# VitorMPCastro/MessyerRaytracer

Measured on AMD Instinct MI355X. Metric: Mrays/s (primary, closest-hit), higher is better.
Workload: dtype f32

## Files before the change

### messyerraytracer_amd/csrc/packet_rows_kernel.h

```cpp
#pragma once

#define RA_LMINX "s20"
#define RA_LMINY "s21"
#define RA_LMINZ "s22"
#define RA_LREF "s23"
#define RA_LMAXX "s24"
#define RA_LMAXY "s25"
#define RA_LMAXZ "s26"
#define RA_RREF "s27"
#define RA_RMINX "s28"
#define RA_RMINY "s29"
#define RA_RMINZ "s30"
#define RA_RMAXX "s32"
#define RA_RMAXY "s33"
#define RA_RMAXZ "s34"
#define RA_MASK "s[60:61]"
#define RA_MASKLO "s60"
#define RA_MASKHI "s61"
#define RA_V0X "s20"
#define RA_V0Y "s21"
#define RA_V0Z "s22"
#define RA_ID "s23"
#define RA_E1X "s24"
#define RA_E1Y "s25"
// ... 179 lines not shown
	"s_branch L_" P "done_%=\n"                                                                                     \
	"L_" P "tri_%=:\n"                                                                                              \
	MRT_ROWS_TRI_STEP(P, RS, POPBIT, CNT_T, ANYHIT_CODE)                                                             \
	"L_" P "done_%=:\n"

#define MRT_ROWS_POP_ISSUE(P, POPBITNO, V0123)                                                                      \
	"s_bitcmp1_b32 %[ev], " POPBITNO "\n"                                                                           \
	"s_cbranch_scc0 L_" P "pi_%=\n"                                                                                 \
	"v_add_u32 " MRT_OP("sp", P) ", -16, " MRT_OP("sp", P) "\n"                                                     \
	"ds_read_b128 " V0123 ", " MRT_OP("sp", P) "\n"                                                                 \
	"L_" P "pi_%=:\n"
#define MRT_ROWS_POP_TAKE(P, RS, POPBITNO, V0, V2, V3)                                                               \
	"s_bitcmp1_b32 %[ev], " POPBITNO "\n"                                                                           \
	"s_cbranch_scc0 L_" P "pt_%=\n"                                                                                 \
	"v_readfirstlane_b32 " MRT_OP("cur", P) ", " V0 "\n"                                                            \
	"v_readfirstlane_b32 " RS##_MASKLO ", " V2 "\n"                                                                  \
	"v_readfirstlane_b32 " RS##_MASKHI ", " V3 "\n"                                                                  \
	"L_" P "pt_%=:\n"

#define MRT_ROWS_CLOBBERS                                                                                             \
	"vcc", "scc", "s20", "s21", "s22", "s23", "s24", "s25", "s26", "s27", "s28", "s29", "s30", "s31", "s32", "s33", \
	"s34", "s35", "s36", "s37", "s38", "s39", "s40", "s41", "s42", "s43", "s44", "s45", "s46", "s47", "s48", "s49", \
	"s50", "s51", "s52", "s53", "s54", "s55", "s56", "s57", "s58", "s59", "s60", "s61", "s62", "s63", "s64", "s65", \
	"s66", "s67", "v50", "v51", "v52", "v53", "v54", "v55", "v56", "v57", "v58", "v59", "v60"

#define MRT_ROWS_OUT(P, S)                                                                                            \
	[cur##P] "+s"(S.cur), [sp##P] "+v"(S.sp), [lim##P] "+v"(S.lim), [bt##P] "+v"(S.bt), [bu##P] "+v"(S.bu),         \
	[bv##P] "+v"(S.bv), [bs##P] "+v"(S.bs), [bi##P] "+v"(S.bi), [mask##P] "+s"(S.mask)
#define MRT_ROWS_IN(P, S)                                                                                             \
	[ox##P] "v"(S.ox), [oy##P] "v"(S.oy), [oz##P] "v"(S.oz), [dx##P] "v"(S.dx), [dy##P] "v"(S.dy), [dz##P] "v"(S.dz), \
	[tmin##P] "v"(S.tmin), [ix##P] "v"(S.ix), [iy##P] "v"(S.iy), [iz##P] "v"(S.iz), [nrx##P] "v"(S.nrx),            \
	[nry##P] "v"(S.nry), [nrz##P] "v"(S.nrz)

struct PacketRegs {
	float ox, oy, oz, dx, dy, dz, tmin;
	float ix, iy, iz, nrx, nry, nrz;
	float lim;
	float bt, bu, bv;
	uint32_t bs, bi;
	uint32_t sp;
	uint32_t cur;
	unsigned long long mask;
};

#define MRT_ROWS_LOOP1(CNT_N, CNT_T, CNT_P, T_PRE, T_POST, ANYHIT_CODE, BX, BY, BZ)                                          \
	asm volatile(                                                                                                   \
		"s_mov_b64 s[60:61], %[maskA]\n"                                                                            \
		"L_loop_%=:\n"                                                                                              \
		"s_lshl_b32 s52, %[curA], 6\n"                                                                              \
		T_PRE                                                                                                       \
		"s_load_dwordx16 s[20:35], %[rows], s52\n"                                                                  \
		"s_waitcnt lgkmcnt(0)\n"                                                                                    \
		T_POST                                                                                                      \
		MRT_ROWS_STEP("A", RA, "1", CNT_N, CNT_T, CNT_P, ANYHIT_CODE, BX, BY, BZ)                                   \
		"s_cmp_eq_u32 %[ev], 0\n"                                                                                   \
		"s_cbranch_scc1 L_loop_%=\n"                                                                                \
		MRT_ROWS_POP_ISSUE("A", "0", "v[50:53]")                                                                    \
		"s_waitcnt lgkmcnt(0)\n"                                                                                    \
		MRT_ROWS_POP_TAKE("A", RA, "0", "v50", "v52", "v53")                                                        \
		"s_mov_b32 %[ev], 0\n"                                                                                      \
		"s_cmp_lg_u32 %[curA], 0x7fffffff\n"                                                                        \
		"s_cbranch_scc1 L_loop_%=\n"                                                                                \
		"s_waitcnt vmcnt(0)\n"                    \
		"s_mov_b64 %[maskA], s[60:61]\n"                                                                            \
		: MRT_ROWS_OUT(A, a), [ev] "+s"(ev), [cntn] "+s"(cnt_n), [cntt] "+s"(cnt_t), [cntw] "+s"(cnt_w), [cntp] "+s"(sp_max) \
		: MRT_ROWS_IN(A, a), [rows] "s"(rows), [qmask] "s"(qmask), [eps] "s"(eps), [vneg] "v"(vneg)                 \
		: MRT_ROWS_CLOBBERS)

#define MRT_ROWSW_GROUP_SLAB(P, OWN, LM, RM, BX, BY, BZ)                                                              \
	"s_cmp_eq_u64 " OWN ", 0\n"                                                                                     \
	"s_cbranch_scc1 L_" P "skip_%=\n"                             \
	MRT_ROWS_SLAB(P, RA, BX, BY, BZ)                                                                                \
	"v_cmp_le_f32_e64 " LM ", v50, v53\n"                                                                           \
	"v_cmp_le_f32_e64 " RM ", v56, v52\n"                                                                           \
	"L_" P "sdone_%=:\n"
#define MRT_ROWSW_GROUP_SKIP(P, LM, RM)                                                                               \
	"L_" P "skip_%=:\n"                                                                                             \
	"s_mov_b64 " LM ", 0\n"                                                                                         \
	"s_mov_b64 " RM ", 0\n"                                                                                         \
	"s_branch L_" P "sdone_%=\n"

#define MRT_ROWSW_ANYHIT(P) \
	"v_cndmask_b32_e64 " MRT_OP("lim", P) ", " MRT_OP("lim", P) ", %[vneg], s[54:55]\n"
#define MRT_ROWSW_ANYDONE                                                                                             \
	"v_cmp_neq_f32_e64 s[56:57], %[limA], %[vneg]\n"                                                                \
	"v_cmp_neq_f32_e64 s[58:59], %[limB], %[vneg]\n"                                                                \
	"s_or_b64 s[56:57], s[56:57], s[58:59]\n"                                                                       \
	"s_cbranch_scc1 L_goon_%=\n"                                                                                    \
	"s_mov_b32 %[curA], 0x7fffffff\n"                                                                               \
	"s_branch L_exit_%=\n"                                                                                          \
	"L_goon_%=:\n"

#ifndef MRT_ROWS_KPREFETCH
#define MRT_ROWS_KPREFETCH 1
#endif
#if MRT_ROWS_KPREFETCH
#define MRT_ROWSW_KPREFETCH                                                                                           \
	"s_lshl_b32 s48, " RA_LREF ", 6\n"                                                                               \
	"s_lshl_b32 s49, " RA_RREF ", 6\n"                                                                               \
	"s_load_dword s64, %[rows], s48\n"                                                                              \
	"s_load_dword s65, %[rows], s49\n"
#define MRT_ROWSW_FARPREFETCH ""
#else
#define MRT_ROWSW_KPREFETCH ""
#define MRT_ROWSW_FARPREFETCH                                                                                         \
	"v_lshlrev_b32 v55, 6, v54\n"                                       \
	"global_load_dword v60, v55, %[rows]\n"
#endif

#define MRT_ROWS_LOOPW(CNT_N, CNT_T, CNT_P, ANYA, ANYB, ANYDONE, BX, BY, BZ)                                                 \
	asm volatile(                                                                                                   \
		"s_mov_b64 s[60:61], %[maskA]\n"                                                                            \
		"s_mov_b64 s[62:63], %[maskB]\n"                                                                            \
		"L_loop_%=:\n"                                                                                              \
		"s_lshl_b32 s52, %[curA], 6\n"                                                                              \
		"s_load_dwordx16 s[20:35], %[rows], s52\n"                                                                  \
		"s_waitcnt lgkmcnt(0)\n"                                                                                    \
		"s_bitcmp1_b32 %[curA], 31\n"                                                                               \
		"s_cbranch_scc1 L_tri_%=\n"                                                                                 \
		CNT_N                                                                                                       \
		MRT_ROWSW_KPREFETCH                                                                                         \
		MRT_ROWSW_GROUP_SLAB("A", "s[60:61]", "s[36:37]", "s[38:39]", BX, BY, BZ)                                   \
		MRT_ROWSW_GROUP_SLAB("B", "s[62:63]", "s[40:41]", "s[42:43]", BX, BY, BZ)                                   \
		"s_or_b64 s[44:45], s[36:37], s[40:41]\n"                     \
		"s_cbranch_scc0 L_lmiss_%=\n"                                                                               \
		"s_or_b64 vcc, s[38:39], s[42:43]\n"                                              \
		"s_cbranch_scc0 L_onlyl_%=\n"                                                                               \
		      \
		"v_cmp_lt_f32_e64 s[46:47], v50, v56\n"                                           \
		"s_bitcmp1_b32 s46, 0\n"                                                                                    \
		"s_cselect_b32 s53, " RA_RREF ", " RA_LREF "\n"                                                   \
		"s_cselect_b32 %[curA], " RA_LREF ", " RA_RREF "\n"                                               \
		"s_cselect_b64 s[50:51], s[38:39], s[36:37]\n"                 \
		"s_cselect_b64 s[58:59], s[42:43], s[40:41]\n"                                                              \
		"s_cselect_b64 s[60:61], s[36:37], s[38:39]\n"                                        \
		"s_cselect_b64 s[62:63], s[40:41], s[42:43]\n"                                                              \
		"v_mov_b32 v50, s50\n"                                                                                      \
		"v_mov_b32 v51, s51\n"                                                                                      \
		"v_mov_b32 v52, s58\n"                                                                                      \
		"v_mov_b32 v53, s59\n"                                                                                      \
		"v_mov_b32 v54, s53\n"                                                                                      \
		"ds_write_b128 %[spA], v[50:53]\n"                                                                          \
		"ds_write_b32 %[spA], v54 offset:16\n"                                                                      \
		"v_add_u32 %[spA], 32, %[spA]\n"                                                                            \
		CNT_P                                                                                                       \
		MRT_ROWSW_FARPREFETCH                                                                                       \
		"s_branch L_loop_%=\n"                                                                                      \
		"L_onlyl_%=:\n"                                                                                             \
		"s_mov_b32 %[curA], " RA_LREF "\n"                                                                          \
		"s_mov_b64 s[60:61], s[36:37]\n"                                                                            \
		"s_mov_b64 s[62:63], s[40:41]\n"                                                                            \
		"s_branch L_loop_%=\n"                                                                                      \
		"L_lmiss_%=:\n"                                                                                             \
		"s_or_b64 vcc, s[38:39], s[42:43]\n"                                                                        \
		"s_cbranch_scc0 L_pop_%=\n"                                                                                 \
		"s_mov_b32 %[curA], " RA_RREF "\n"                                                                          \
		"s_mov_b64 s[60:61], s[38:39]\n"                                                                            \
		"s_mov_b64 s[62:63], s[42:43]\n"                                                                            \
		"s_branch L_loop_%=\n"                                                                                      \
		"L_tri_%=:\n"                                                                                               \
		CNT_T                                                                                                       \
		"s_cmp_eq_u64 s[60:61], 0\n"                                                                                \
		"s_cbranch_scc1 L_Atnext_%=\n"                                                                              \
		MRT_ROWS_TRI_TEST("A", RA, "s[60:61]", "%[curA]", ANYA)                                                     \
		"s_cmp_eq_u64 s[62:63], 0\n"                                                                                \
		"s_cbranch_scc1 L_Btnext_%=\n"                                                                              \
		MRT_ROWS_TRI_TEST("B", RA, "s[62:63]", "%[curA]", ANYB)                                                     \
		ANYDONE                                                                                                     \
		"s_bitcmp1_b32 " RA_FLAGS ", 0\n"                                       \
		"s_cbranch_scc1 L_pop_%=\n"                                                                                 \
		"s_add_u32 %[curA], %[curA], 1\n"                                                                           \
		"s_branch L_loop_%=\n"                                                                                      \
		"L_pop_%=:\n"                                                                                               \
		"v_add_u32 %[spA], -32, %[spA]\n"                                                                           \
		"ds_read_b128 v[50:53], %[spA]\n"                                                                           \
		"ds_read_b32 v54, %[spA] offset:16\n"                                                                       \
		"s_waitcnt lgkmcnt(0)\n"                                                                                    \
		"v_readfirstlane_b32 %[curA], v54\n"                                                                        \
		"v_readfirstlane_b32 s60, v50\n"                                                                            \
		"v_readfirstlane_b32 s61, v51\n"                                                                            \
		"v_readfirstlane_b32 s62, v52\n"                                                                            \
		"v_readfirstlane_b32 s63, v53\n"                                                                            \
		"s_cmp_lg_u32 %[curA], 0x7fffffff\n"                                                                        \
		"s_cbranch_scc1 L_loop_%=\n"                                                                                \
		"s_branch L_exit_%=\n"                                                                                      \
		MRT_ROWSW_GROUP_SKIP("A", "s[36:37]", "s[38:39]")                                                           \
		MRT_ROWSW_GROUP_SKIP("B", "s[40:41]", "s[42:43]")                                                           \
		"L_exit_%=:\n"                                                                                              \
		"s_waitcnt vmcnt(0)\n"                    \
		"s_mov_b64 %[maskA], s[60:61]\n"                                                                            \
		"s_mov_b64 %[maskB], s[62:63]\n"                                                                            \
		: MRT_ROWS_OUT(A, a), [limB] "+v"(b.lim), [btB] "+v"(b.bt), [buB] "+v"(b.bu), [bvB] "+v"(b.bv),             \
		  [bsB] "+v"(b.bs), [biB] "+v"(b.bi), [maskB] "+s"(b.mask), [cntn] "+s"(cnt_n), [cntt] "+s"(cnt_t), [cntp] "+s"(sp_max) \
		: MRT_ROWS_IN(A, a), MRT_ROWS_IN(B, b), [rows] "s"(rows), [qmask] "s"(qmask), [eps] "s"(eps), [vneg] "v"(vneg) \
		: MRT_ROWS_CLOBBERS)


#define MRT_ROWS_SLAB1(P, RS, SIDE, TE, BX, BY, BZ, MASK)                                                             \
	"v_fma_f32 v51, " MRT_NEAR_##BX(RS, X, SIDE) ", " MRT_OP("ix", P) ", " MRT_OP("nrx", P) "\n"                      \
	"v_fma_f32 v52, " MRT_NEAR_##BY(RS, Y, SIDE) ", " MRT_OP("iy", P) ", " MRT_OP("nry", P) "\n"                      \
	"v_fma_f32 v53, " MRT_NEAR_##BZ(RS, Z, SIDE) ", " MRT_OP("iz", P) ", " MRT_OP("nrz", P) "\n"                      \
	"v_fma_f32 v54, " MRT_FAR_##BX(RS, X, SIDE) ", " MRT_OP("ix", P) ", " MRT_OP("nrx", P) "\n"                       \
	"v_fma_f32 v55, " MRT_FAR_##BY(RS, Y, SIDE) ", " MRT_OP("iy", P) ", " MRT_OP("nry", P) "\n"                       \
	"v_fma_f32 v57, " MRT_FAR_##BZ(RS, Z, SIDE) ", " MRT_OP("iz", P) ", " MRT_OP("nrz", P) "\n"                       \
	"v_max_f32 v53, v53, " MRT_OP("tmin", P) "\n"                                                                   \
	"v_min_f32 v57, v57, " MRT_OP("lim", P) "\n"                                                                    \
	"v_max3_f32 " TE ", v51, v52, v53\n"                                                                            \
	"v_min3_f32 v54, v54, v55, v57\n"                                                                               \
	"v_cmp_le_f32_e64 " MASK ", " TE ", v54\n"

#define MRT_ROWSC_CHILD(SIDE, TE, CULLBITS, MA, MB, BX, BY, BZ)                                                       \
	"s_and_b32 s48, s44, " CULLBITS "\n"                                 \
	"s_cbranch_scc1 L_cull" #SIDE "_%=\n"                                                                           \
	"s_cmp_eq_u64 s[60:61], 0\n"                                                                                    \
	"s_cbranch_scc1 L_" #SIDE "A0_%=\n"                                                                             \
	MRT_ROWS_SLAB1("A", RA, SIDE, TE, BX, BY, BZ, MA)                                                               \
	"L_" #SIDE "A1_%=:\n"                                                                                           \
	"s_cmp_eq_u64 s[62:63], 0\n"                                                                                    \
	"s_cbranch_scc1 L_" #SIDE "B0_%=\n"                                                                             \
	MRT_ROWS_SLAB1("B", RA, SIDE, TE, BX, BY, BZ, MB)                                                               \
	"L_" #SIDE "B1_%=:\n"
#define MRT_ROWSC_CHILD_OOL(SIDE, MA, MB)                                                                             \
	"L_cull" #SIDE "_%=:\n"                                                                                         \
	MRT_ROWSC_CNT_CULL                                                                                              \
	"s_mov_b64 " MA ", 0\n"                                                                                         \
	"s_mov_b64 " MB ", 0\n"                                                                                         \
	"s_branch L_" #SIDE "B1_%=\n"                                                                                   \
	"L_" #SIDE "A0_%=:\n"                                                                                           \
	"s_mov_b64 " MA ", 0\n"                                                                                         \
	"s_branch L_" #SIDE "A1_%=\n"                                                                                   \
	"L_" #SIDE "B0_%=:\n"                                                                                           \
	"s_mov_b64 " MB ", 0\n"                                                                                         \
	"s_branch L_" #SIDE "B1_%=\n"
#define MRT_ROWSC_CNT_CULL ""

#define MRT_ROWSC_VLOAD(VDST, REF)                                                                                   \
	"v_lshl_add_u32 v62, " REF ", 6, %[cvo]\n"                                                                      \
	"global_load_dword " VDST ", v62, %[rows]\n"

#ifndef MRT_ROWSC_KPF
#define MRT_ROWSC_KPF 0
#endif
#if MRT_ROWSC_KPF
#define MRT_ROWSC_KPREFETCH                                                                                           \
	"s_lshl_b32 s46, " RA_LREF ", 6\n"                                                                               \
	"s_lshl_b32 s47, " RA_RREF ", 6\n"                                                                               \
	"s_load_dword s64, %[rows], s46\n"                                                                              \
	"s_load_dword s65, %[rows], s47\n"
#else
#define MRT_ROWSC_KPREFETCH ""
#endif
#define MRT_ROWS_LOOPC(CNT_N, CNT_T, CNT_P, ANYA, ANYB, ANYDONE, BX, BY, BZ)                                          \
	asm volatile(                                                                                                   \
		"s_mov_b64 s[60:61], %[maskA]\n"                                                                            \
		"s_mov_b64 s[62:63], %[maskB]\n"                                                                            \
		"L_vload_%=:\n"                                     \
		MRT_ROWSC_VLOAD("v60", "%[curA]")                                                                           \
		"s_mov_b64 s[66:67], 0\n"                                                                                   \
		"L_loop_%=:\n"                                                                                              \
		"s_lshl_b32 s52, %[curA], 6\n"                                                                              \
		"s_load_dwordx16 s[20:35], %[rows], s52\n"                                                                  \
		"s_waitcnt lgkmcnt(0)\n"                                                                                    \
		"s_bitcmp1_b32 %[curA], 31\n"                                                                               \
		"s_cbranch_scc1 L_tri_%=\n"                                                                                 \
		CNT_N                                                                                                       \
		"s_waitcnt vmcnt(0)\n"                      \
		"v_cndmask_b32_e64 v58, v60, v61, s[66:67]\n"                                                               \
		"v_mul_f32 v58, v58, %[cw]\n"                                                                               \
		MRT_ROWSC_VLOAD("v60", RA_LREF)            \
		"v_add_f32_dpp v59, v58, v58 row_shr:1 row_mask:0xf bank_mask:0xf bound_ctrl:1\n"  \
		MRT_ROWSC_VLOAD("v61", RA_RREF)                                                                             \
		"v_add_f32_dpp v58, v59, v59 row_shr:2 row_mask:0xf bank_mask:0xf bound_ctrl:1\n"                           \
		"s_nop 1\n"                                                                                                 \
		"v_add_f32_dpp v59, v58, v58 row_shr:4 row_mask:0xf bank_mask:0xf bound_ctrl:1\n"                           \
		"v_cmp_lt_f32_e64 s[44:45], v59, %[ccc]\n"  \
		MRT_ROWSC_KPREFETCH                                                                                         \
		"s_or_b32 s44, s44, s45\n"                                                                                  \
		MRT_ROWSC_CHILD(L, "v50", "0x00800080", "s[36:37]", "s[40:41]", BX, BY, BZ)                                 \
// ... 36 lines not shown
		"s_mov_b64 s[62:63], s[42:43]\n"                                                                            \
		"s_mov_b64 s[66:67], -1\n"                                                                                  \
		"s_branch L_loop_%=\n"                                                                                      \
		"L_tri_%=:\n"                                                                                               \
		CNT_T                                                                                                       \
		"s_cmp_eq_u64 s[60:61], 0\n"                                                                                \
		"s_cbranch_scc1 L_Atnext_%=\n"                                                                              \
		MRT_ROWS_TRI_TEST("A", RA, "s[60:61]", "%[curA]", ANYA)                                                     \
		"s_cmp_eq_u64 s[62:63], 0\n"                                                                                \
		"s_cbranch_scc1 L_Btnext_%=\n"                                                                              \
		MRT_ROWS_TRI_TEST("B", RA, "s[62:63]", "%[curA]", ANYB)                                                     \
		ANYDONE                                                                                                     \
		"s_bitcmp1_b32 " RA_FLAGS ", 0\n"                                       \
		"s_cbranch_scc1 L_pop_%=\n"                                                                                 \
		"s_add_u32 %[curA], %[curA], 1\n"                                                                           \
		"s_branch L_loop_%=\n"                                                                                      \
		"L_pop_%=:\n"                                                                                               \
		"v_add_u32 %[spA], -32, %[spA]\n"                                                                           \
		"ds_read_b128 v[50:53], %[spA]\n"                                                                           \
		"ds_read_b32 v54, %[spA] offset:16\n"                                                                       \
		"s_waitcnt lgkmcnt(0)\n"                                                                                    \
		"v_readfirstlane_b32 %[curA], v54\n"                                                                        \
		"v_readfirstlane_b32 s60, v50\n"                                                                            \
		"v_readfirstlane_b32 s61, v51\n"                                                                            \
		"v_readfirstlane_b32 s62, v52\n"                                                                            \
		"v_readfirstlane_b32 s63, v53\n"                                                                            \
		"s_cmp_lg_u32 %[curA], 0x7fffffff\n"                                                                        \
		"s_cbranch_scc1 L_vload_%=\n"                                                                               \
		"s_branch L_exit_%=\n"                                                                                      \
		MRT_ROWSC_CHILD_OOL(L, "s[36:37]", "s[40:41]")                                                              \
		MRT_ROWSC_CHILD_OOL(R, "s[38:39]", "s[42:43]")                                                              \
		"L_exit_%=:\n"                                                                                              \
		"s_waitcnt vmcnt(0)\n"                 \
		"s_mov_b64 %[maskA], s[60:61]\n"                                                                            \
		"s_mov_b64 %[maskB], s[62:63]\n"                                                                            \
		: MRT_ROWS_OUT(A, a), [limB] "+v"(b.lim), [btB] "+v"(b.bt), [buB] "+v"(b.bu), [bvB] "+v"(b.bv),             \
		  [bsB] "+v"(b.bs), [biB] "+v"(b.bi), [maskB] "+s"(b.mask), [cntn] "+s"(cnt_n), [cntt] "+s"(cnt_t), [cntp] "+s"(sp_max) \
		: MRT_ROWS_IN(A, a), MRT_ROWS_IN(B, b), [rows] "s"(rows), [qmask] "s"(qmask),                                \
		  [eps] "s"(eps), [vneg] "v"(vneg), [cw] "v"(cull.w), [ccc] "v"(cull.cc), [cvo] "v"(cull.voff)               \
		: MRT_ROWS_CLOBBERS, "v61", "v62")

struct CullRegs {
	float w;
	float cc;
	uint32_t voff;
};

#define MRT_ROWS_T_PRE "s_memtime s[64:65]\n s_waitcnt lgkmcnt(0)\n"
#define MRT_ROWS_T_POST "s_memtime s[66:67]\n s_waitcnt lgkmcnt(0)\n s_sub_u32 s64, s66, s64\n s_add_u32 %[cntw], %[cntw], s64\n"
#define MRT_ROWS_CNT_N "s_add_u32 %[cntn], %[cntn], 1\n"
#define MRT_ROWS_CNT_P "v_readfirstlane_b32 s52, %[spA]\n s_max_u32 %[cntp], %[cntp], s52\n"
#define MRT_ROWS_CNT_T "s_add_u32 %[cntt], %[cntt], 1\n"

__device__ __forceinline__ void rows_uniform(PacketRegs &s)
{
	s.cur = __builtin_amdgcn_readfirstlane(s.cur);
	const uint32_t lo = __builtin_amdgcn_readfirstlane((uint32_t)s.mask), hi = __builtin_amdgcn_readfirstlane((uint32_t)(s.mask >> 32));
	s.mask = ((unsigned long long)hi << 32) | lo;
}

template <int OCT, bool ANY_HIT, bool COUNT>
__device__ __forceinline__ void rows_walk_one(const float4 *rows, uint32_t qmask, PacketRegs &a, uint32_t &cnt_n, uint32_t &cnt_t, uint32_t &cnt_w, uint32_t &sp_max)
{
	const float eps = 1e-8f, vneg = -FLT_MAX;
	uint32_t ev = 0u;
#define MRT_W1(O, BX, BY, BZ)                                                                                         \
	if (OCT == O) {                                                                                                 \
		if (COUNT) { if (ANY_HIT) MRT_ROWS_LOOP1(MRT_ROWS_CNT_N, MRT_ROWS_CNT_T, MRT_ROWS_CNT_P, MRT_ROWS_T_PRE, MRT_ROWS_T_POST, MRT_ROWS_ANYHIT("A", "4"), BX, BY, BZ); \
			else MRT_ROWS_LOOP1(MRT_ROWS_CNT_N, MRT_ROWS_CNT_T, MRT_ROWS_CNT_P, MRT_ROWS_T_PRE, MRT_ROWS_T_POST, MRT_ROWS_NEAREST("A"), BX, BY, BZ); } \
		else { if (ANY_HIT) MRT_ROWS_LOOP1("", "", "", "", "", MRT_ROWS_ANYHIT("A", "4"), BX, BY, BZ);              \
			else MRT_ROWS_LOOP1("", "", "", "", "", MRT_ROWS_NEAREST("A"), BX, BY, BZ); }                           \
	}
	MRT_W1(0, 0, 0, 0) MRT_W1(1, 1, 0, 0) MRT_W1(2, 0, 1, 0) MRT_W1(3, 1, 1, 0) MRT_W1(4, 0, 0, 1) MRT_W1(5, 1, 0, 1) MRT_W1(6, 0, 1, 1) MRT_W1(7, 1, 1, 1)
#undef MRT_W1
	rows_uniform(a);
	cnt_n = __builtin_amdgcn_readfirstlane(cnt_n); cnt_t = __builtin_amdgcn_readfirstlane(cnt_t); cnt_w = __builtin_amdgcn_readfirstlane(cnt_w);
	sp_max = __builtin_amdgcn_readfirstlane(sp_max);
}

template <int OCT, bool ANY_HIT, bool COUNT>
__device__ __forceinline__ void rows_walk_wide(const float4 *rows, uint32_t qmask, PacketRegs &a, PacketRegs &b, uint32_t &cnt_n, uint32_t &cnt_t, uint32_t &sp_max)
{
	const float eps = 1e-8f, vneg = -FLT_MAX;
#define MRT_WW(O, BX, BY, BZ)                                                                                         \
	if (OCT == O) {                                                                                                 \
		if (COUNT) { if (ANY_HIT) MRT_ROWS_LOOPW(MRT_ROWS_CNT_N, MRT_ROWS_CNT_T, MRT_ROWS_CNT_P, MRT_ROWSW_ANYHIT("A"), MRT_ROWSW_ANYHIT("B"), MRT_ROWSW_ANYDONE, BX, BY, BZ); \
			else MRT_ROWS_LOOPW(MRT_ROWS_CNT_N, MRT_ROWS_CNT_T, MRT_ROWS_CNT_P, MRT_ROWS_NEAREST("A"), MRT_ROWS_NEAREST("B"), "", BX, BY, BZ); } \
		else { if (ANY_HIT) MRT_ROWS_LOOPW("", "", "", MRT_ROWSW_ANYHIT("A"), MRT_ROWSW_ANYHIT("B"), MRT_ROWSW_ANYDONE, BX, BY, BZ); \
			else MRT_ROWS_LOOPW("", "", "", MRT_ROWS_NEAREST("A"), MRT_ROWS_NEAREST("B"), "", BX, BY, BZ); }        \
	}
	MRT_WW(0, 0, 0, 0) MRT_WW(1, 1, 0, 0) MRT_WW(2, 0, 1, 0) MRT_WW(3, 1, 1, 0) MRT_WW(4, 0, 0, 1) MRT_WW(5, 1, 0, 1) MRT_WW(6, 0, 1, 1) MRT_WW(7, 1, 1, 1)
#undef MRT_WW
	rows_uniform(a);
	cnt_n = __builtin_amdgcn_readfirstlane(cnt_n); cnt_t = __builtin_amdgcn_readfirstlane(cnt_t);
	sp_max = __builtin_amdgcn_readfirstlane(sp_max);
}

template <int OCT, bool ANY_HIT, bool COUNT>
__device__ __forceinline__ void rows_walk_cull(const float4 *rows, uint32_t qmask, PacketRegs &a, PacketRegs &b, const CullRegs &cull, uint32_t &cnt_n, uint32_t &cnt_t, uint32_t &sp_max)
{
	const float eps = 1e-8f, vneg = -FLT_MAX;
#define MRT_WC(O, BX, BY, BZ)                                                                                         \
	if (OCT == O) {                                                                                                 \
		if (COUNT) { if (ANY_HIT) MRT_ROWS_LOOPC(MRT_ROWS_CNT_N, MRT_ROWS_CNT_T, MRT_ROWS_CNT_P, MRT_ROWSW_ANYHIT("A"), MRT_ROWSW_ANYHIT("B"), MRT_ROWSW_ANYDONE, BX, BY, BZ); \
			else MRT_ROWS_LOOPC(MRT_ROWS_CNT_N, MRT_ROWS_CNT_T, MRT_ROWS_CNT_P, MRT_ROWS_NEAREST("A"), MRT_ROWS_NEAREST("B"), "", BX, BY, BZ); } \
		else { if (ANY_HIT) MRT_ROWS_LOOPC("", "", "", MRT_ROWSW_ANYHIT("A"), MRT_ROWSW_ANYHIT("B"), MRT_ROWSW_ANYDONE, BX, BY, BZ); \
			else MRT_ROWS_LOOPC("", "", "", MRT_ROWS_NEAREST("A"), MRT_ROWS_NEAREST("B"), "", BX, BY, BZ); }        \
	}
	MRT_WC(0, 0, 0, 0) MRT_WC(1, 1, 0, 0) MRT_WC(2, 0, 1, 0) MRT_WC(3, 1, 1, 0) MRT_WC(4, 0, 0, 1) MRT_WC(5, 1, 0, 1) MRT_WC(6, 0, 1, 1) MRT_WC(7, 1, 1, 1)
#undef MRT_WC
	rows_uniform(a);
	cnt_n = __builtin_amdgcn_readfirstlane(cnt_n); cnt_t = __builtin_amdgcn_readfirstlane(cnt_t);
	sp_max = __builtin_amdgcn_readfirstlane(sp_max);
}

__device__ __forceinline__ CullRegs cull_setup(const RayRegs &ra, const RayRegs &rb, bool valid_a, bool valid_b, unsigned long long part_a,
		unsigned long long part_b, float scene_abs_max, uint32_t lane)
{
	CullRegs c;
	c.w = 0.0f; c.cc = -__builtin_inff(); c.voff = (lane & 15u) * 4u;
	const bool corners = (part_a & 1ull) && (part_a >> 56 & 1ull) && (part_b >> 7 & 1ull) && (part_b >> 63 & 1ull);
	if (!corners) return c;
#define MRT_RL(v, l) __builtin_bit_cast(float, __builtin_amdgcn_readlane(__builtin_bit_cast(int, v), l))
	const float ox = MRT_RL(ra.ox, 0), oy = MRT_RL(ra.oy, 0), oz = MRT_RL(ra.oz, 0);
	const float tl[3] = { MRT_RL(ra.dx, 0), MRT_RL(ra.dy, 0), MRT_RL(ra.dz, 0) }, bl[3] = { MRT_RL(ra.dx, 56), MRT_RL(ra.dy, 56), MRT_RL(ra.dz, 56) };
	const float tr[3] = { MRT_RL(rb.dx, 7), MRT_RL(rb.dy, 7), MRT_RL(rb.dz, 7) }, br[3] = { MRT_RL(rb.dx, 63), MRT_RL(rb.dy, 63), MRT_RL(rb.dz, 63) };
	float cen[3] = { tl[0] + tr[0] + bl[0] + br[0], tl[1] + tr[1] + bl[1] + br[1], tl[2] + tr[2] + bl[2] + br[2] };
	const float cl = __builtin_sqrtf(cen[0] * cen[0] + cen[1] * cen[1] + cen[2] * cen[2]);
	if (!(cl > 0.0f)) return c;
	cen[0] /= cl; cen[1] /= cl; cen[2] /= cl;
	const uint32_t k = lane >> 4;
	const float *pa = k == 0u ? tl : (k == 1u ? tr : (k == 2u ? br : bl)), *pb = k == 0u ? tr : (k == 1u ? br : (k == 2u ? bl : tl));
	float n[3] = { pa[1] * pb[2] - pa[2] * pb[1], pa[2] * pb[0] - pa[0] * pb[2], pa[0] * pb[1] - pa[1] * pb[0] };
	const float nl = __builtin_sqrtf(n[0] * n[0] + n[1] * n[1] + n[2] * n[2]);
	bool ok = nl > 0.0f;
	const float inv = ok ? 1.0f / nl : 0.0f;
	n[0] *= inv; n[1] *= inv; n[2] *= inv;
	if (n[0] * cen[0] + n[1] * cen[1] + n[2] * cen[2] < 0.0f) { n[0] = -n[0]; n[1] = -n[1]; n[2] = -n[2]; }
	const float push = 5e-5f;
	n[0] += push * cen[0]; n[1] += push * cen[1]; n[2] += push * cen[2];
	bool inside = true;
	for (int q = 0; q < 4; q++) {
		const float qx = MRT_RL(n[0], 16 * q), qy = MRT_RL(n[1], 16 * q), qz = MRT_RL(n[2], 16 * q);
		const float da = qx * ra.dx + qy * ra.dy + qz * ra.dz, la = __builtin_sqrtf(ra.dx * ra.dx + ra.dy * ra.dy + ra.dz * ra.dz);
		const float db = qx * rb.dx + qy * rb.dy + qz * rb.dz, lb = __builtin_sqrtf(rb.dx * rb.dx + rb.dy * rb.dy + rb.dz * rb.dz);
		if (valid_a && !(da >= 1e-5f * la)) inside = false;
		if (valid_b && !(db >= 1e-5f * lb)) inside = false;
	}
#undef MRT_RL
	if (valid_a && !(ra.ox == ox && ra.oy == oy && ra.oz == oz && ra.t_min >= 0.0f)) inside = false;
	if (valid_b && !(rb.ox == ox && rb.oy == oy && rb.oz == oz && rb.t_min >= 0.0f)) inside = false;
	ok = ok && __builtin_isfinite(n[0]) && __builtin_isfinite(n[1]) && __builtin_isfinite(n[2]);
	const bool planes_ok = (__ballot(ok) & 0x0001000100010001ull) == 0x0001000100010001ull;
	if (__ballot(!inside) != 0ull || !planes_ok) return c;
	const float n1 = __builtin_fabsf(n[0]) + __builtin_fabsf(n[1]) + __builtin_fabsf(n[2]);
	const float o1 = __builtin_fabsf(ox) + __builtin_fabsf(oy) + __builtin_fabsf(oz);
	const float err = 8.0f * 5.9604645e-8f * n1 * (scene_abs_max + o1);
	const float cc = (n[0] * ox + n[1] * oy + n[2] * oz) - err;
	if (__ballot(!__builtin_isfinite(cc)) != 0ull) return c;
	const uint32_t d = lane & 15u, axis = d & 3u;
	const bool is_max = (d >> 2 & 1u) != 0u;
	const float na = axis == 0u ? n[0] : (axis == 1u ? n[1] : n[2]);
	c.w = (axis < 3u && ((na >= 0.0f) == is_max)) ? na : 0.0f;
	c.cc = (d == 7u || d == 15u) ? cc : -__builtin_inff();
	return c;
}

__device__ __forceinline__ void rows_init(PacketRegs &s, const RayRegs &r, bool takes_part, uint32_t sp)
{
	s.ox = r.ox; s.oy = r.oy; s.oz = r.oz; s.dx = r.dx; s.dy = r.dy; s.dz = r.dz; s.tmin = r.t_min;
	s.ix = safe_inv(r.dx); s.iy = safe_inv(r.dy); s.iz = safe_inv(r.dz);
	s.nrx = -(r.ox * s.ix); s.nry = -(r.oy * s.iy); s.nrz = -(r.oz * s.iz);
	s.bt = r.t_max; s.bu = 0.0f; s.bv = 0.0f; s.bs = 0xFFFFFFFFu; s.bi = 0xFFFFFFFFu;
	s.lim = (!takes_part || r.t_min >= r.t_max) ? -FLT_MAX : r.t_max;
	s.sp = sp; s.cur = 0u; s.mask = 0ull;
}

__device__ __forceinline__ int rows_octant(const RayRegs &r, bool part, unsigned long long &part_mask)
{
	part_mask = __ballot(part);
	const unsigned long long sx = __ballot(part && safe_inv(r.dx) < 0.0f), sy = __ballot(part && safe_inv(r.dy) < 0.0f),
			sz = __ballot(part && safe_inv(r.dz) < 0.0f);
	const bool uniform = (sx == 0ull || sx == part_mask) && (sy == 0ull || sy == part_mask) && (sz == 0ull || sz == part_mask);
	return uniform ? ((sx ? 1 : 0) | (sy ? 2 : 0) | (sz ? 4 : 0)) : 8;
}

#ifndef MRT_ROWS_WPE
#define MRT_ROWS_WPE 8
#endif
template <bool ANY_HIT, bool COUNT, int PACKETS, int WG, bool CULL = false>
__global__ __launch_bounds__(WG) __attribute__((amdgpu_waves_per_eu(MRT_ROWS_WPE, 8))) void trace_packet_rows_kernel(const TraceParams p)
{
	__shared__ __attribute__((aligned(16))) uint32_t wave_stack[WG / MRT_WAVE][PACKETS][(MRT_PACKET_STACK + 1) * 4];
	if (skip_launch(p)) return;
	uint32_t block = blockIdx.x;
	if (p.xcd_swizzle) {
		const uint32_t per = gridDim.x >> 3;
		if (block < (per << 3)) block = (block & 7u) * per + (block >> 3);
	}
	const uint32_t wave = threadIdx.x / MRT_WAVE, lane = threadIdx.x & (MRT_WAVE - 1);
	const uint32_t wave_s = __builtin_amdgcn_readfirstlane(wave), block_s = block;
	const uint64_t g_a = (((uint64_t)block * (WG / MRT_WAVE) + wave) * PACKETS) * MRT_WAVE + lane, g_b = g_a + MRT_WAVE;
	uint64_t idx = 0; uint32_t px = 0, py = 0;
	const bool valid_a = lane_ray_index_g(p, g_a, idx, px, py);
	RayRegs ra = {0.0f, 0.0f, 0.0f, 0.0f, 0.0f, 0.0f, 1.0f, 0.0f}, rb = ra;
	if (valid_a) load_ray(p, idx, px, py, ra);
	bool valid_b = false;
	if (PACKETS == 2) {
		valid_b = lane_ray_index_g(p, g_b, idx, px, py);
		if (valid_b) load_ray(p, idx, px, py, rb);
	}
	if (__ballot(valid_a || valid_b) == 0ull) return;

	const float4 *rows = reinterpret_cast<const float4 *>(p.row_array);
	uint32_t *stack_a = wave_stack[wave][0], *stack_b = wave_stack[wave][PACKETS - 1];
	*(volatile uint32_t *)&stack_a[0] = kSentinel;
	if (PACKETS == 2) *(volatile uint32_t *)&stack_b[0] = kSentinel;
	PacketRegs A, B;
	rows_init(A, ra, valid_a, (uint32_t)(uintptr_t)(__attribute__((address_space(3))) uint32_t *)(stack_a + 4));
	rows_init(B, rb, valid_b, (uint32_t)(uintptr_t)(__attribute__((address_space(3))) uint32_t *)(stack_b + 4));

	unsigned long long part_a = 0ull, part_b = 0ull;
	const int oct_a = rows_octant(ra, valid_a, part_a);
	const int oct_b = PACKETS == 2 ? rows_octant(rb, valid_b, part_b) : 8;
	uint32_t cnt_n = 0u, cnt_t = 0u;
	uint32_t cnt_w = 0u;
	uint32_t sp_wide = 0u, sp_one = 0u;
	if (p.tile_cost != nullptr && lane == 0u) note_tile_start(p, g_a);
	if (COUNT) *(volatile unsigned long long *)&stack_a[2] = __builtin_amdgcn_s_memtime();
	bool done_a = part_a == 0ull, done_b = part_b == 0ull;
	if (PACKETS == 2 && !done_a && !done_b && oct_a == oct_b && oct_a != 8) {
		*(volatile uint32_t *)&stack_a[4] = kSentinel;
		A.sp += 16u;
		A.mask = part_a; B.mask = part_b;
		if (CULL) {
			const CullRegs cull = cull_setup(ra, rb, valid_a, valid_b, part_a, part_b, p.scene_abs_max, lane);
#define MRT_RWC(O) case O: rows_walk_cull<O, ANY_HIT, COUNT>(rows, p.query_mask, A, B, cull, cnt_n, cnt_t, sp_wide); break;
			switch (oct_a) { MRT_RWC(0) MRT_RWC(1) MRT_RWC(2) MRT_RWC(3) MRT_RWC(4) MRT_RWC(5) MRT_RWC(6) MRT_RWC(7) }
#undef MRT_RWC
		} else {
#define MRT_RW2(O) case O: rows_walk_wide<O, ANY_HIT, COUNT>(rows, p.query_mask, A, B, cnt_n, cnt_t, sp_wide); break;
		switch (oct_a) { MRT_RW2(0) MRT_RW2(1) MRT_RW2(2) MRT_RW2(3) MRT_RW2(4) MRT_RW2(5) MRT_RW2(6) MRT_RW2(7) }
#undef MRT_RW2
		}
		done_a = done_b = true;
	}
#define MRT_RW1(O, S) case O: rows_walk_one<O, ANY_HIT, COUNT>(rows, p.query_mask, S, cnt_n, cnt_t, cnt_w, sp_one); break;
	if (!done_a && oct_a != 8) { switch (oct_a) { MRT_RW1(0, A) MRT_RW1(1, A) MRT_RW1(2, A) MRT_RW1(3, A) MRT_RW1(4, A) MRT_RW1(5, A) MRT_RW1(6, A) MRT_RW1(7, A) } done_a = true; }
	if (PACKETS == 2 && !done_b && oct_b != 8) { switch (oct_b) { MRT_RW1(0, B) MRT_RW1(1, B) MRT_RW1(2, B) MRT_RW1(3, B) MRT_RW1(4, B) MRT_RW1(5, B) MRT_RW1(6, B) MRT_RW1(7, B) } done_b = true; }
#undef MRT_RW1
	uint32_t slot_a = A.bs == 0xFFFFFFFFu ? 0xFFFFFFFFu : A.bs - p.n_nodes, slot_b = B.bs == 0xFFFFFFFFu ? 0xFFFFFFFFu : B.bs - p.n_nodes;
	if (!done_a) {
		uint32_t nn = 0, nt = 0, nd = 0;
		A.bt = ra.t_max;
		packet_traverse<8, ANY_HIT, COUNT>(p, ra, stack_a, A.bt, A.bu, A.bv, slot_a, nn, nt, nd, 0u, 0u, nullptr, !valid_a);
		if (COUNT) { cnt_n += __builtin_amdgcn_readfirstlane(nn); cnt_t += __builtin_amdgcn_readfirstlane(nt); }
	}
	if (PACKETS == 2 && !done_b) {
		uint32_t nn = 0, nt = 0, nd = 0;
		B.bt = rb.t_max;
		packet_traverse<8, ANY_HIT, COUNT>(p, rb, stack_b, B.bt, B.bu, B.bv, slot_b, nn, nt, nd, 0u, 0u, nullptr, !valid_b);
		if (COUNT) { cnt_n += __builtin_amdgcn_readfirstlane(nn); cnt_t += __builtin_amdgcn_readfirstlane(nt); }
	}

	{
		const uint32_t lane2 = __builtin_amdgcn_mbcnt_hi(~0u, __builtin_amdgcn_mbcnt_lo(~0u, 0u));
		const uint64_t h_a = (((uint64_t)block_s * (WG / MRT_WAVE) + wave_s) * PACKETS) * MRT_WAVE + lane2;
		uint64_t idx2 = 0; uint32_t px2 = 0, py2 = 0;
		if (lane_ray_index_g(p, h_a, idx2, px2, py2)) finish_ray(p, idx2, ra, A.bt, A.bu, A.bv, slot_a);
		if (PACKETS == 2 && lane_ray_index_g(p, h_a + MRT_WAVE, idx2, px2, py2)) finish_ray(p, idx2, rb, B.bt, B.bu, B.bv, slot_b);
		if (p.tile_cost != nullptr && lane2 == 0u) note_tile_cost(p, h_a);
	}
	const unsigned long long t_start = COUNT ? *(volatile unsigned long long *)&stack_a[2] : 0ull;
	if (COUNT && lane == 0u && (p.count_mode != 2u || (blockIdx.x & 15u) == 0u)) {
		atomicAdd(&p.counters[kCntFetchWaitCycles], (unsigned long long)cnt_w);
		atomicAdd(&p.counters[kCntWaveCycles], __builtin_amdgcn_s_memtime() - t_start);
		atomicAdd(&p.counters[kCntWaves], 1ull);
	}
	if (COUNT && p.count_mode != 2u) {
		const uint32_t base = (uint32_t)(uintptr_t)(__attribute__((address_space(3))) uint32_t *)stack_a;
		const uint32_t e_wide = sp_wide > base ? (sp_wide - base) / 32u : 0u, e_one = sp_one > base ? ((sp_one - base) % 1040u) / 16u : 0u;
		atomicMax(&p.counters[kCntMaxStack], (unsigned long long)(e_wide > e_one ? e_wide : e_one));
	}
	if (COUNT && p.count_mode != 2u) {
		if (valid_a) packet_count(p, cnt_n, cnt_t, 0u, slot_a != 0xFFFFFFFFu, part_a | part_b);
		if (PACKETS == 2 && valid_b) { atomicAdd(&p.counters[kCntRays], 1ull); if (slot_b != 0xFFFFFFFFu) atomicAdd(&p.counters[kCntHits], 1ull); }
	}
}
```

Baseline: 8671.

## Keep wide-walk traversal stack in VGPR lanes and issue node fetch early

Replaces the LDS-based traversal stack of the two-packet wide walk with a lane-indexed stack in v60..v63 plus one extra VGPR, pushed with v_writelane and popped with v_readlane using m0 as the stack pointer. This avoids ds_write/ds_read round trips and the lgkmcnt wait on every pop. It also issues the next node's scalar load at each branch point, before the loop header, so the fetch overlaps the remaining bookkeeping. The cost is extra VGPR pressure, a stack depth limited to 64 entries by the wave width, and saving and restoring m0.

```diff
diff --git a/messyerraytracer_amd/csrc/packet_rows_kernel.h b/messyerraytracer_amd/csrc/packet_rows_kernel.h
--- a/messyerraytracer_amd/csrc/packet_rows_kernel.h
+++ b/messyerraytracer_amd/csrc/packet_rows_kernel.h
@@ -285,6 +285,7 @@
 
 #define MRT_ROWSW_ANYHIT(P) \
 	"v_cndmask_b32_e64 " MRT_OP("lim", P) ", " MRT_OP("lim", P) ", %[vneg], s[54:55]\n"
+#define MRT_ROWSW_VNEG , [vneg] "v"(vneg)
 #define MRT_ROWSW_ANYDONE                                                                                             \
 	"v_cmp_neq_f32_e64 s[56:57], %[limA], %[vneg]\n"                                                                \
 	"v_cmp_neq_f32_e64 s[58:59], %[limB], %[vneg]\n"                                                                \
@@ -311,13 +312,121 @@
 	"global_load_dword v60, v55, %[rows]\n"
 #endif
 
-#define MRT_ROWS_LOOPW(CNT_N, CNT_T, CNT_P, ANYA, ANYB, ANYDONE, BX, BY, BZ)                                                 \
+#ifndef MRT_ROWS_LANESTACK
+#define MRT_ROWS_LANESTACK 1
+#endif
+#ifndef MRT_ROWS_EARLYFETCH
+#define MRT_ROWS_EARLYFETCH 1
+#endif
+#ifndef MRT_ROWS_POPPREFETCH
+#define MRT_ROWS_POPPREFETCH 0
+#endif
+#if MRT_ROWS_POPPREFETCH && !MRT_ROWS_LANESTACK
+#error "MRT_ROWS_POPPREFETCH reads the top of the lane stack: it needs MRT_ROWS_LANESTACK=1"
+#endif
+#if MRT_ROWS_POPPREFETCH
+#define MRT_ROWSW_POPPREFETCH                                                                                         \
+	"s_bitcmp1_b32 " RA_FLAGS ", 0\n"                                                                                \
+	"s_cbranch_scc0 L_npp_%=\n"                                                                                     \
+	"s_sub_u32 s49, m0, 1\n"                                   \
+	"s_cbranch_scc1 L_npp_%=\n"                                                                                     \
+	"v_readlane_b32 s48, %[stk], s49\n"                                                                             \
+	"s_lshl_b32 s48, s48, 6\n"                                                                                      \
+	"s_load_dword s49, %[rows], s48\n"                                                                              \
+	"L_npp_%=:\n"
+#else
+#define MRT_ROWSW_POPPREFETCH ""
+#endif
+#if MRT_ROWS_LANESTACK && !MRT_ROWS_KPREFETCH
+#error "MRT_ROWS_LANESTACK keeps the stack in v60..v63: it needs MRT_ROWS_KPREFETCH=1 (v60 is the far-child prefetch's destination otherwise)"
+#endif
+#define MRT_ROWSW_FETCH                                                                                               \
+	"s_lshl_b32 s52, %[curA], 6\n"                                                                                  \
+	"s_load_dwordx16 s[20:35], %[rows], s52\n"
+#if MRT_ROWS_EARLYFETCH
+#define MRT_ROWSW_FETCH_EARLY MRT_ROWSW_FETCH
+#define MRT_ROWSW_FETCH_LATE ""
+#else
+#define MRT_ROWSW_FETCH_EARLY ""
+#define MRT_ROWSW_FETCH_LATE MRT_ROWSW_FETCH
+#endif
+#if MRT_ROWS_LANESTACK
+#define MRT_ROWSW_ENTER                                                                                               \
+	"s_mov_b32 %[m0s], m0\n"                                                                                        \
+	"s_mov_b32 m0, 0\n"
+#define MRT_ROWSW_PUSH                                                                                                \
+	"v_writelane_b32 v60, s50, m0\n"                                                                                \
+	"v_writelane_b32 v61, s51, m0\n"                                                                                \
+	"v_writelane_b32 v62, s58, m0\n"                                                                                \
+	"v_writelane_b32 v63, s59, m0\n"                                                                                \
+	"v_writelane_b32 %[stk], s53, m0\n"                                                                             \
+	"s_add_u32 m0, m0, 1\n"
+#define MRT_ROWSW_POP                                                                                                 \
+	"s_sub_u32 m0, m0, 1\n"                                                  \
+	"s_cbranch_scc1 L_exit_%=\n"                                                                                    \
+	"v_readlane_b32 %[curA], %[stk], m0\n"                                                                          \
+	MRT_ROWSW_FETCH_EARLY                                                                                           \
+	"v_readlane_b32 s60, v60, m0\n"                                                                                 \
+	"v_readlane_b32 s61, v61, m0\n"                                                                                 \
+	"v_readlane_b32 s62, v62, m0\n"                                                                                 \
+	"v_readlane_b32 s63, v63, m0\n"                                                                                 \
+	"s_branch L_loop_%=\n"
+#define MRT_ROWSW_LEAVE                                                                                               \
+	"s_waitcnt lgkmcnt(0)\n"                                                                                        \
+	"s_mov_b32 m0, %[m0s]\n"                                                                                        \
+	"s_mov_b32 %[curA], 0x7fffffff\n"
+#define MRT_ROWSW_CNT_P "s_max_u32 %[cntp], %[cntp], m0\n"
+#define MRT_ROWSW_STACK_OUT [stk] "=&v"(stk), [m0s] "=&s"(m0s)
+#define MRT_ROWSW_STACK_CLOBBERS , "v61", "v62", "v63"
+#define MRT_ROWSW_STACK_VARS uint32_t stk, m0s;
+#else
+#define MRT_ROWSW_ENTER ""
+#define MRT_ROWSW_PUSH                                                                                                \
+	"v_mov_b32 v50, s50\n"                                                                                          \
+	"v_mov_b32 v51, s51\n"                                                                                          \
+	"v_mov_b32 v52, s58\n"                                                                                          \
+	"v_mov_b32 v53, s59\n"                                                                                          \
+	"v_mov_b32 v54, s53\n"                                                                                          \
+	"ds_write_b128 %[spA], v[50:53]\n"                                                                              \
+	"ds_write_b32 %[spA], v54 offset:16\n"                                                                          \
+	"v_add_u32 %[spA], 32, %[spA]\n"
+#if MRT_ROWS_EARLYFETCH
+#define MRT_ROWSW_POP_TAIL                                                                                            \
+	"s_cbranch_scc0 L_exit_%=\n"                                                                                    \
+	MRT_ROWSW_FETCH                                                                                                 \
+	"s_branch L_loop_%=\n"
+#else
+#define MRT_ROWSW_POP_TAIL                                                                                            \
+	"s_cbranch_scc1 L_loop_%=\n"                                                                                    \
+	"s_branch L_exit_%=\n"
+#endif
+#define MRT_ROWSW_POP                                                                                                 \
+	"v_add_u32 %[spA], -32, %[spA]\n"                                                                               \
+	"ds_read_b128 v[50:53], %[spA]\n"                                                                               \
+	"ds_read_b32 v54, %[spA] offset:16\n"                                                                           \
+	"s_waitcnt lgkmcnt(0)\n"                                                                                        \
+	"v_readfirstlane_b32 %[curA], v54\n"                                                                            \
+	"v_readfirstlane_b32 s60, v50\n"                                                                                \
+	"v_readfirstlane_b32 s61, v51\n"                                                                                \
+	"v_readfirstlane_b32 s62, v52\n"                                                                                \
+	"v_readfirstlane_b32 s63, v53\n"                                                                                \
+	"s_cmp_lg_u32 %[curA], 0x7fffffff\n"                                                                            \
+	MRT_ROWSW_POP_TAIL
+#define MRT_ROWSW_LEAVE ""
+#define MRT_ROWSW_CNT_P "v_readfirstlane_b32 s44, %[spA]\n s_max_u32 %[cntp], %[cntp], s44\n"
+#define MRT_ROWSW_STACK_OUT [spA] "+v"(a.sp)
+#define MRT_ROWSW_STACK_CLOBBERS
+#define MRT_ROWSW_STACK_VARS
+#endif
+
+#define MRT_ROWS_LOOPW(CNT_N, CNT_T, CNT_P, ANYA, ANYB, ANYDONE, VNEG_IN, BX, BY, BZ)                                                 \
 	asm volatile(                                                                                                   \
 		"s_mov_b64 s[60:61], %[maskA]\n"                                                                            \
 		"s_mov_b64 s[62:63], %[maskB]\n"                                                                            \
+		MRT_ROWSW_ENTER                                                                                             \
+		MRT_ROWSW_FETCH_EARLY                                                                                       \
 		"L_loop_%=:\n"                                                                                              \
-		"s_lshl_b32 s52, %[curA], 6\n"                                                                              \
-		"s_load_dwordx16 s[20:35], %[rows], s52\n"                                                                  \
+		MRT_ROWSW_FETCH_LATE                                                                                        \
 		"s_waitcnt lgkmcnt(0)\n"                                                                                    \
 		"s_bitcmp1_b32 %[curA], 31\n"                                                                               \
 		"s_cbranch_scc1 L_tri_%=\n"                                                                                 \
@@ -338,19 +447,14 @@
 		"s_cselect_b64 s[58:59], s[42:43], s[40:41]\n"                                                              \
 		"s_cselect_b64 s[60:61], s[36:37], s[38:39]\n"                                        \
 		"s_cselect_b64 s[62:63], s[40:41], s[42:43]\n"                                                              \
-		"v_mov_b32 v50, s50\n"                                                                                      \
-		"v_mov_b32 v51, s51\n"                                                                                      \
-		"v_mov_b32 v52, s58\n"                                                                                      \
-		"v_mov_b32 v53, s59\n"                                                                                      \
-		"v_mov_b32 v54, s53\n"                                                                                      \
-		"ds_write_b128 %[spA], v[50:53]\n"                                                                          \
-		"ds_write_b32 %[spA], v54 offset:16\n"                                                                      \
-		"v_add_u32 %[spA], 32, %[spA]\n"                                                                            \
+		MRT_ROWSW_FETCH_EARLY                                                                                       \
+		MRT_ROWSW_PUSH                                                                                              \
 		CNT_P                                                                                                       \
 		MRT_ROWSW_FARPREFETCH                                                                                       \
 		"s_branch L_loop_%=\n"                                                                                      \
 		"L_onlyl_%=:\n"                                                                                             \
 		"s_mov_b32 %[curA], " RA_LREF "\n"                                                                          \
+		MRT_ROWSW_FETCH_EARLY                                                                                       \
 		"s_mov_b64 s[60:61], s[36:37]\n"                                                                            \
 		"s_mov_b64 s[62:63], s[40:41]\n"                                                                            \
 		"s_branch L_loop_%=\n"                                                                                      \
@@ -358,11 +462,13 @@
 		"s_or_b64 vcc, s[38:39], s[42:43]\n"                                                                        \
 		"s_cbranch_scc0 L_pop_%=\n"                                                                                 \
 		"s_mov_b32 %[curA], " RA_RREF "\n"                                                                          \
+		MRT_ROWSW_FETCH_EARLY                                                                                       \
 		"s_mov_b64 s[60:61], s[38:39]\n"                                                                            \
 		"s_mov_b64 s[62:63], s[42:43]\n"                                                                            \
 		"s_branch L_loop_%=\n"                                                                                      \
 		"L_tri_%=:\n"                                                                                               \
 		CNT_T                                                                                                       \
+		MRT_ROWSW_POPPREFETCH                                                                                       \
 		"s_cmp_eq_u64 s[60:61], 0\n"                                                                                \
 		"s_cbranch_scc1 L_Atnext_%=\n"                                                                              \
 		MRT_ROWS_TRI_TEST("A", RA, "s[60:61]", "%[curA]", ANYA)                                                     \
@@ -373,30 +479,23 @@
 		"s_bitcmp1_b32 " RA_FLAGS ", 0\n"                                       \
 		"s_cbranch_scc1 L_pop_%=\n"                                                                                 \
 		"s_add_u32 %[curA], %[curA], 1\n"                                                                           \
+		MRT_ROWSW_FETCH_EARLY                                                                                       \
 		"s_branch L_loop_%=\n"                                                                                      \
 		"L_pop_%=:\n"                                                                                               \
-		"v_add_u32 %[spA], -32, %[spA]\n"                                                                           \
-		"ds_read_b128 v[50:53], %[spA]\n"                                                                           \
-		"ds_read_b32 v54, %[spA] offset:16\n"                                                                       \
-		"s_waitcnt lgkmcnt(0)\n"                                                                                    \
-		"v_readfirstlane_b32 %[curA], v54\n"                                                                        \
-		"v_readfirstlane_b32 s60, v50\n"                                                                            \
-		"v_readfirstlane_b32 s61, v51\n"                                                                            \
-		"v_readfirstlane_b32 s62, v52\n"                                                                            \
-		"v_readfirstlane_b32 s63, v53\n"                                                                            \
-		"s_cmp_lg_u32 %[curA], 0x7fffffff\n"                                                                        \
-		"s_cbranch_scc1 L_loop_%=\n"                                                                                \
-		"s_branch L_exit_%=\n"                                                                                      \
+		MRT_ROWSW_POP                                                                                               \
 		MRT_ROWSW_GROUP_SKIP("A", "s[36:37]", "s[38:39]")                                                           \
 		MRT_ROWSW_GROUP_SKIP("B", "s[40:41]", "s[42:43]")                                                           \
 		"L_exit_%=:\n"                                                                                              \
 		"s_waitcnt vmcnt(0)\n"                    \
+		MRT_ROWSW_LEAVE                                                                                             \
 		"s_mov_b64 %[maskA], s[60:61]\n"                                                                            \
 		"s_mov_b64 %[maskB], s[62:63]\n"                                                                            \
-		: MRT_ROWS_OUT(A, a), [limB] "+v"(b.lim), [btB] "+v"(b.bt), [buB] "+v"(b.bu), [bvB] "+v"(b.bv),             \
+		: [curA] "+s"(a.cur), MRT_ROWSW_STACK_OUT, [limA] "+v"(a.lim), [btA] "+v"(a.bt), [buA] "+v"(a.bu),          \
+		  [bvA] "+v"(a.bv), [bsA] "+v"(a.bs), [biA] "+v"(a.bi), [maskA] "+s"(a.mask),                               \
+		  [limB] "+v"(b.lim), [btB] "+v"(b.bt), [buB] "+v"(b.bu), [bvB] "+v"(b.bv),                                 \
 		  [bsB] "+v"(b.bs), [biB] "+v"(b.bi), [maskB] "+s"(b.mask), [cntn] "+s"(cnt_n), [cntt] "+s"(cnt_t), [cntp] "+s"(sp_max) \
-		: MRT_ROWS_IN(A, a), MRT_ROWS_IN(B, b), [rows] "s"(rows), [qmask] "s"(qmask), [eps] "s"(eps), [vneg] "v"(vneg) \
-		: MRT_ROWS_CLOBBERS)
+		: MRT_ROWS_IN(A, a), MRT_ROWS_IN(B, b), [rows] "s"(rows), [qmask] "s"(qmask), [eps] "s"(eps) VNEG_IN \
+		: MRT_ROWS_CLOBBERS MRT_ROWSW_STACK_CLOBBERS)
 
 
 #define MRT_ROWS_SLAB1(P, RS, SIDE, TE, BX, BY, BZ, MASK)                                                             \
@@ -599,12 +698,13 @@
 __device__ __forceinline__ void rows_walk_wide(const float4 *rows, uint32_t qmask, PacketRegs &a, PacketRegs &b, uint32_t &cnt_n, uint32_t &cnt_t, uint32_t &sp_max)
 {
 	const float eps = 1e-8f, vneg = -FLT_MAX;
+	MRT_ROWSW_STACK_VARS
 #define MRT_WW(O, BX, BY, BZ)                                                                                         \
 	if (OCT == O) {                                                                                                 \
-		if (COUNT) { if (ANY_HIT) MRT_ROWS_LOOPW(MRT_ROWS_CNT_N, MRT_ROWS_CNT_T, MRT_ROWS_CNT_P, MRT_ROWSW_ANYHIT("A"), MRT_ROWSW_ANYHIT("B"), MRT_ROWSW_ANYDONE, BX, BY, BZ); \
-			else MRT_ROWS_LOOPW(MRT_ROWS_CNT_N, MRT_ROWS_CNT_T, MRT_ROWS_CNT_P, MRT_ROWS_NEAREST("A"), MRT_ROWS_NEAREST("B"), "", BX, BY, BZ); } \
-		else { if (ANY_HIT) MRT_ROWS_LOOPW("", "", "", MRT_ROWSW_ANYHIT("A"), MRT_ROWSW_ANYHIT("B"), MRT_ROWSW_ANYDONE, BX, BY, BZ); \
-			else MRT_ROWS_LOOPW("", "", "", MRT_ROWS_NEAREST("A"), MRT_ROWS_NEAREST("B"), "", BX, BY, BZ); }        \
+		if (COUNT) { if (ANY_HIT) MRT_ROWS_LOOPW(MRT_ROWS_CNT_N, MRT_ROWS_CNT_T, MRT_ROWSW_CNT_P, MRT_ROWSW_ANYHIT("A"), MRT_ROWSW_ANYHIT("B"), MRT_ROWSW_ANYDONE, MRT_ROWSW_VNEG, BX, BY, BZ); \
+			else MRT_ROWS_LOOPW(MRT_ROWS_CNT_N, MRT_ROWS_CNT_T, MRT_ROWSW_CNT_P, MRT_ROWS_NEAREST("A"), MRT_ROWS_NEAREST("B"), "", , BX, BY, BZ); } \
+		else { if (ANY_HIT) MRT_ROWS_LOOPW("", "", "", MRT_ROWSW_ANYHIT("A"), MRT_ROWSW_ANYHIT("B"), MRT_ROWSW_ANYDONE, MRT_ROWSW_VNEG, BX, BY, BZ); \
+			else MRT_ROWS_LOOPW("", "", "", MRT_ROWS_NEAREST("A"), MRT_ROWS_NEAREST("B"), "", , BX, BY, BZ); }        \
 	}
 	MRT_WW(0, 0, 0, 0) MRT_WW(1, 1, 0, 0) MRT_WW(2, 0, 1, 0) MRT_WW(3, 1, 1, 0) MRT_WW(4, 0, 0, 1) MRT_WW(5, 1, 0, 1) MRT_WW(6, 0, 1, 1) MRT_WW(7, 1, 1, 1)
 #undef MRT_WW
@@ -747,8 +847,10 @@
 	if (COUNT) *(volatile unsigned long long *)&stack_a[2] = __builtin_amdgcn_s_memtime();
 	bool done_a = part_a == 0ull, done_b = part_b == 0ull;
 	if (PACKETS == 2 && !done_a && !done_b && oct_a == oct_b && oct_a != 8) {
-		*(volatile uint32_t *)&stack_a[4] = kSentinel;
-		A.sp += 16u;
+		if (CULL || !MRT_ROWS_LANESTACK) {
+			*(volatile uint32_t *)&stack_a[4] = kSentinel;
+			A.sp += 16u;
+		}
 		A.mask = part_a; B.mask = part_b;
 		if (CULL) {
 			const CullRegs cull = cull_setup(ra, rb, valid_a, valid_b, part_a, part_b, p.scene_abs_max, lane);
@@ -796,7 +898,8 @@
 	}
 	if (COUNT && p.count_mode != 2u) {
 		const uint32_t base = (uint32_t)(uintptr_t)(__attribute__((address_space(3))) uint32_t *)stack_a;
-		const uint32_t e_wide = sp_wide > base ? (sp_wide - base) / 32u : 0u, e_one = sp_one > base ? ((sp_one - base) % 1040u) / 16u : 0u;
+		const uint32_t e_lds = sp_wide > base + 32u ? (sp_wide - base) / 32u - 1u : 0u, e_wide = (MRT_ROWS_LANESTACK && !CULL) ? sp_wide : e_lds;
+		const uint32_t e_one = sp_one > base ? ((sp_one - base) % 1040u) / 16u : 0u;
 		atomicMax(&p.counters[kCntMaxStack], (unsigned long long)(e_wide > e_one ? e_wide : e_one));
 	}
 	if (COUNT && p.count_mode != 2u) {
```

After: 8709, median of 3. About the same (+0.4%).
